# worldbench/lidarcrafter

Measured on AMD Instinct MI355X. Metric: denoising-steps/sec, nuScenes 32×1024 range image, 1/2/4/8 GPU, higher is better.
Workload: dtype f16x2-split MFMA, fp32 accumulate (fp32-class accuracy)

## Files before the change

### include/lidarcrafter_hip.h

```cpp
#ifndef LIDARCRAFTER_HIP_H
#define LIDARCRAFTER_HIP_H

#include <stdint.h>

#ifdef __cplusplus
extern "C" {
#endif

#define LC_OK 0
#define LC_EINVAL (-1)
#define LC_EUNSUP (-2)

typedef void* lc_stream_t;

int lc_abi_version(void);
int lc_device_arch(char* buf, int buflen);
int lc_load_code_objects(void);

int64_t lc_packed_conv_weight_elems(int Co, int Ci, int ks);
int lc_pack_conv_weight(const float* w_oihw, float* wp, int Co, int Ci, int ks, lc_stream_t s);
int lc_conv2d_ring_fwd(const float* x, int64_t x_bs, const float* wp, const float* bias,
                       const float* res, int64_t res_bs, float* y, int64_t y_bs,
                       int B, int Ci, int Co, int H, int W, int ks, float out_scale,
                       int tile_cfg , lc_stream_t s);
// ... 142 lines not shown
int lc_hdit_rmsnorm_fwd(const float* x, int64_t x_bs, int64_t x_cs, const float* f, int64_t f_bs, int mode, float* y,
                        int64_t y_bs, int64_t y_cs, int B, int C, int L, float eps, lc_stream_t s);
int lc_hdit_geglu_fwd(const float* x, int64_t x_bs, float* y, int64_t y_bs, int B, int mid, int L, lc_stream_t s);
int lc_hdit_qk_prep_fwd(float* q, int64_t q_bs, int64_t q_cs, float* k, int64_t k_bs, int64_t k_cs, const float* scale,
                        const float* cos_t, const float* sin_t, int B, int heads, int d, int L, lc_stream_t s);
int lc_hdit_na_fwd(const lc_cm_operand* q, const lc_cm_operand* k, const lc_cm_operand* v, float* o, int64_t o_bs,
                   int64_t o_hs, int64_t o_cs, int B, int heads, int d, int h, int w, int kh, int kw, float scale,
                   lc_stream_t s);
int lc_hdit_space_to_depth_fwd(const float* in, int64_t in_bs, float* out, int64_t out_bs, int B, int C, int H, int W,
                               int P1, int P2, lc_stream_t s);
int lc_hdit_depth_to_space_fwd(const float* in, int64_t in_bs, float* out, int64_t out_bs, const float* skip,
                               int64_t skip_bs, const float* alpha, int B, int C, int h, int w, int P1, int P2,
                               lc_stream_t s);
int lc_hdit_tokenize_fwd(const float* x, int64_t x_bs, const float* wt, const float* pe, float* y, int64_t y_bs, int B,
                         int Cin, int C, int H, int W, int P, lc_stream_t s);
int lc_hdit_fourier_fwd(const float* t, const float* freqs, float* y, int M, int half, lc_stream_t s);
int lc_hdit_na_train_fwd(const lc_cm_operand* q, const lc_cm_operand* k, const lc_cm_operand* v, float* o,
                         int64_t o_bs, int64_t o_hs, int64_t o_cs, float* lse, int B, int heads, int d, int h, int w,
                         int kh, int kw, float scale, lc_stream_t s);
int lc_hdit_rmsnorm_bwd(const float* x, int64_t x_bs, int64_t x_cs, const float* f, int64_t f_bs, int mode,
                        const float* dy, int64_t dy_bs, int64_t dy_cs, float* dx, int64_t dx_bs, int64_t dx_cs,
                        float* rs, float* df, int64_t df_bs, int B, int C, int L, float eps, lc_stream_t s);
int lc_hdit_geglu_bwd(const float* x, int64_t x_bs, const float* dy, int64_t dy_bs, float* dx, int64_t dx_bs, int B,
                      int mid, int L, lc_stream_t s);
int lc_hdit_qk_prep_bwd(const float* q, int64_t q_bs, int64_t q_cs, const float* k, int64_t k_bs, int64_t k_cs,
                        const float* gq, int64_t gq_bs, int64_t gq_cs, const float* gk, int64_t gk_bs, int64_t gk_cs,
                        float* dq, int64_t dq_bs, int64_t dq_cs, float* dk, int64_t dk_bs, int64_t dk_cs,
                        const float* scale, const float* cos_t, const float* sin_t, double* part, float* dscale, int B,
                        int heads, int d, int L, lc_stream_t s);
int lc_hdit_na_bwd(const lc_cm_operand* q, const lc_cm_operand* k, const lc_cm_operand* v, const lc_cm_operand* o,
                   const lc_cm_operand* dout, const float* lse, float* dsum, float* dq, float* dk, float* dv, int B,
                   int heads, int d, int h, int w, int kh, int kw, float scale, lc_stream_t s);
int lc_hdit_lerp_bwd(const float* dout, int64_t dout_bs, const float* y, int64_t y_bs, const float* skip,
                     int64_t skip_bs, const float* alpha, float* dskip, int64_t dskip_bs, float* dy, int64_t dy_bs,
                     float* dalpha, int B, int C, int h, int w, int P1, int P2, lc_stream_t s);
int64_t lc_groupnorm_jvp_partials_elems(int B, int C, int H, int W, int G);
int lc_groupnorm_jvp_stats(const float* x, int64_t x_bs, const float* dx, int64_t dx_bs, double* partials, int B, int C,
                           int H, int W, int G, lc_stream_t s);
int lc_groupnorm_jvp_apply_train(const float* x, int64_t x_bs, const float* dx, int64_t dx_bs, const double* partials,
                                 const float* gamma, const float* beta, const float* scale, const float* shift,
                                 const float* dscale, const float* dshift, int64_t ss_bs, float* y, int64_t y_bs,
                                 float* dy, int64_t dy_bs, int B, int C, int H, int W, int G, float eps, int act_silu,
                                 float* mean_rstd_out, float* amax_out, float* damax_out, lc_stream_t s);
int lc_qk_norm_cm_jvp(const float* x, int64_t x_bs, int64_t x_cs, const float* dx, int64_t dx_bs, int64_t dx_cs,
                      const float* g, float* y, int64_t y_bs, int64_t y_cs, float* dy, int64_t dy_bs, int64_t dy_cs,
                      int B, int heads, int d, int L, lc_stream_t s);
int64_t lc_qk_norm_cm_bwd_partials(int B, int heads, int L);
int lc_qk_norm_cm_bwd(const float* x, int64_t x_bs, int64_t x_cs, const float* gy, int64_t gy_bs, int64_t gy_cs,
                      const float* g, float* gx, int64_t gx_bs, int64_t gx_cs, double* dg_partials, float* dg, int B,
                      int heads, int d, int L, lc_stream_t s);
int lc_attention_jvp_fwd(const float* q, const float* k, const float* v, const float* dq, const float* dk,
                         const float* dv, float* o, float* lse, float* dout, int BH, int Lq, int Lk, int dqk, int dv_ch,
                         float scale, lc_stream_t s);
int lc_conv1x1_f16x2_ps_qkv_fwd(const void* x_split, const void* wp_hi, const void* wp_lo, const float* bias, float* q,
                                int64_t q_bs, void* kv, int B, int Ci, int C, int H, int W, int Lk1, const float* wmeta,
                                lc_conv_range* range, lc_stream_t s);
int64_t lc_attention_units_elems(int B, int heads, int Lk0, int Lk1);
int lc_attention_pack_units(const lc_cm_operand* src, void* kv, int B, int heads, int L, int Lk0, int Lk1, int d,
                            int cb0, int key0, int which, lc_stream_t s);
int lc_attention_units_fwd(const lc_cm_operand* q, const lc_cm_operand* q_pos, const void* kv, float* o,
                           int64_t o_bs, int64_t o_hs, int64_t o_cs, int B, int heads, int Lq, int Lk0, int Lk1,
                           int dqk, int dpos, int dv, float scale, lc_stream_t s);
int lc_attention_train_fwd(const float* q, const float* k, const float* v, float* o, float* lse, int BH, int Lq,
                           int Lk, int dqk, int dv, float scale, int f16x2, float* qkv_amax, lc_stream_t s);
int lc_attention_bwd(const float* q, const float* k, const float* v, const float* o, const float* dout,
                     const float* lse, float* dsum_scratch, float* dq, float* dk, float* dv, int BH, int Lq, int Lk,
                     int dqk, int dv_ch, float scale, lc_stream_t s);
int lc_attention_bwd_f16x2(const float* q, const float* k, const float* v, const float* o, const float* dout,
                           const float* lse, float* dsum_scratch, float* dq, float* dk, float* dv, int BH, int Lq,
                           int Lk, int dqk, int dv_ch, float scale, const float* qkv_amax, lc_stream_t s);

int lc_pstep_fwd(const float* x_t, int64_t xt_bs, const float* pred, int64_t pred_bs,
                 const float* noise, int64_t noise_bs, const float* coef, float* x_s,
                 int64_t xs_bs, int B, int64_t n, int objective, int mode, lc_stream_t s);

int lc_gate_bias_act(const float* x, int64_t x_bs, const float* gate_logit, const float* bias,
                     int64_t gb_bs, const float* res, int64_t res_bs, float* y, int64_t y_bs,
                     int B, int C, int N, int act, lc_stream_t s);

int64_t lc_fir_down2_split_units(int B, int C, int H, int W);
int lc_fir_down2_prefilter_split(const float* x, int64_t x_bs, void* y_split, int B, int C, int H, int W,
                                 lc_conv_range* range, lc_stream_t s);
int64_t lc_conv2d_ring_s2_stats_slots(int Ho, int Wo);
int lc_conv2d_ring_s2_f16x2_ps_fwd(const void* x_split, const void* wp_hi, const void* wp_lo, const float* bias, float* y,
                                   int64_t y_bs, int B, int Ci, int Co, int Ho, int Wo, float out_scale,
                                   float* gn_ostats_out, int gn_ostats_unit, const float* wmeta, lc_conv_range* range,
                                   lc_stream_t s);

int64_t lc_calibrate_mfma_f16(const void* operands, int blocks, int iters, float* sink, lc_stream_t s);
int lc_calibrate_stream_copy(const float* src, float* dst, int64_t n, lc_stream_t s);

int lc_copy_strided(const float* x, int64_t x_bs, float* y, int64_t y_bs, int B, int64_t n,
                    lc_stream_t s);
int lc_add_scale(const float* a, int64_t a_bs, const float* b, int64_t b_bs, float* y,
                 int64_t y_bs, int B, int64_t n, float scale, lc_stream_t s);

int64_t lc_conv2d_ring_wgrad_scratch_elems(int B, int Ci, int Co, int H, int W, int ks);
int lc_conv2d_ring_wgrad(const float* x, int64_t x_bs, const float* dy, int64_t dy_bs, float* scratch,
                         float* dw , float* dbias , int B, int Ci,
                         int Co, int H, int W, int ks, int accumulate, lc_stream_t s);
int lc_conv2d_ring_wgrad_f16x2(const float* x, int64_t x_bs, const float* dy, int64_t dy_bs,
                               const lc_conv_range* x_range, const lc_conv_range* dy_range,
                               float* scratch, float* dw, float* dbias, int B, int Ci, int Co, int H,
                               int W, int ks, int accumulate, lc_stream_t s);
int lc_groupnorm_meanrstd(const float* x, int64_t x_bs, const double* partials, float* mean_rstd,
                          int B, int C, int H, int W, int G, float eps, lc_stream_t s);
int lc_groupnorm_bwd(const float* x, int64_t x_bs, const float* dy, int64_t dy_bs,
                     const float* mean_rstd, const float* gamma, const float* beta, const float* scale,
                     const float* shift, int64_t ss_bs, double* rows, float* dx, int64_t dx_bs, int B,
                     int C, int H, int W, int G, int act_silu, lc_stream_t s);
int lc_groupnorm_bwd_train(const float* x, int64_t x_bs, const float* dy, int64_t dy_bs,
                           const float* mean_rstd, const float* gamma, const float* beta, const float* scale,
                           const float* shift, int64_t ss_bs, double* rows, float* dx, int64_t dx_bs,
                           float* dgamma, float* dbeta, float* dscale, float* dshift, int B, int C, int H, int W,
                           int G, int act_silu, float* amax_out, lc_stream_t s);

int lc_bev_occupancy_accumulate(const float* pts, int pt_stride, int N, float x0, float x1, float y0,
                                float y1, float voxel, int min_bound_x, int min_bound_y, int nx,
                                int ny, int stamp, int32_t* stamps, float* grid, lc_stream_t s);
int64_t lc_sparse_quantize_scratch_bytes(int N, int D);
int lc_sparse_quantize(const float* coords, int N, int D, float vx, float vy, float vz, void* scratch,
                       int32_t* out_coords, int64_t* out_index, int64_t* out_inverse,
                       uint64_t* out_count, lc_stream_t s);

int lc_project_points(const float* points, int N, int H, int W, double fov_up_deg,
                      double fov_down_deg, float min_depth, float max_depth, uint64_t* zbuf,
                      float* image, int32_t* winner, int32_t* cells, int elev_f64, lc_stream_t s);
int lc_project_workspace_init(uint64_t* zbuf, int n_cells, lc_stream_t s);
int lc_project_points_ws(const float* points, int N, int H, int W, double fov_up_deg,
                         double fov_down_deg, float min_depth, float max_depth, uint64_t* zbuf,
                         float* image, int32_t* winner, int32_t* cells, int elev_f64, lc_stream_t s);
int lc_project_points_f64(const double* points, int N, int H, int W, double fov_up_deg,
                          double fov_down_deg, double min_depth, double max_depth, uint64_t* zbuf,
                          int32_t* winner, float* image, lc_stream_t s);

int lc_points_in_boxes_mask(const float* boxes, int n_boxes, const float* pts, int n_pts,
                            float margin, int32_t* out_mask, lc_stream_t s);
int lc_points_in_boxes_index(const float* boxes, const float* pts, int B, int n_boxes, int n_pts,
                             float margin, int32_t* out_idx, lc_stream_t s);

int lc_range_postprocess(const float* sample, int64_t sample_bs, const float* ray_angles,
                         float* out, int B, int H, int W, int depth_format, float min_depth,
                         float max_depth, lc_stream_t s);
int lc_condition_preprocess(const float* condition_mask, int64_t cm_bs, float* out, int64_t out_bs,
                            int B, int H, int W, int num_classes, int depth_format,
                            float min_depth, float max_depth, lc_stream_t s);

int64_t lc_layout_scratch_bytes(int B, int T);
int lc_layout_condition(const void* boxes, int boxes_f64, int box_stride, const int32_t* n_valid,
                        int B, int T, int H, int W, double fov_up_deg, double fov_down_deg,
                        void* scratch, float* corners_2d, float* condition_mask,
                        float* loss_weight_map, lc_stream_t s);

int lc_roiaware_pool3d_fwd(const float* rois, const float* pts, const float* pts_feature,
                           int n_boxes, int n_pts, int channels, int out_x, int out_y, int out_z,
                           int max_pts_each_voxel, int pool_method, int32_t* pts_mask_scratch,
                           int32_t* pts_idx_of_voxels, int32_t* argmax, float* pooled,
                           lc_stream_t s);
int lc_roiaware_pool3d_bwd(const int32_t* pts_idx_of_voxels, const int32_t* argmax,
                           const float* grad_out, float* grad_in, int n_boxes, int channels,
                           int out_x, int out_y, int out_z, int max_pts_each_voxel,
                           int pool_method, lc_stream_t s);

int lc_transform_points(const float* pts, int N, const double* T16_host, float* out, lc_stream_t s);
int lc_transform_points_f64(const float* pts, int N, const double* T16_host, int rot_f32,
                            double* out, lc_stream_t s);
// ... 79 lines not shown
```

### lidarcrafter_amd/_lib.py

```python
from __future__ import annotations

import ctypes as C
import os

from .build import LIB

i32, i64, f32, f64, vp = C.c_int, C.c_int64, C.c_float, C.c_double, C.c_void_p


class CmOperand(C.Structure):
    _fields_ = [("p", vp), ("bs", i64), ("hs", i64), ("cs", i64)]


_op = C.POINTER(CmOperand)


class OctStats(C.Structure):
    _fields_ = [("p", vp), ("channels", i32), ("slots", i32), ("unit", i32)]


_os = C.POINTER(OctStats)


class GnStatsInput(C.Structure):
# ... 35 lines not shown
    "lc_groupnorm_apply_split": (i32, [vp, i64, vp, vp, vp, vp, vp, i64, vp, i32, i32, i32, i32, i32,
                                       f32, i32, vp, vp]),
    "lc_groupnorm_apply_os_split": (i32, [vp, i64, _os, _os, vp, vp, vp, vp, i64, vp, i32, i32, i32,
                                          i32, i32, f32, i32, vp, vp]),
    "lc_conv1x1_f16x2_ps_fwd": (i32, [vp, vp, vp, vp, vp, i64, vp, i64, i32, i32, i32, i32, i32, f32, vp, vp, vp]),
    "lc_conv2d_ring_f16x2_ps_fwd": (i32, [vp, vp, vp, vp, vp, i64, vp, i64, i32, i32, i32, i32, i32,
                                          f32, i32, vp, i32, vp, i32, vp, vp, vp]),
    "lc_range_from_tensor": (i32, [vp, i64, i32, i64, vp, vp]),
    "lc_splitk_stats_slots": (i64, [i32, i32]),
    "lc_splitk_reduce": (i32, [vp, i32, vp, vp, i64, vp, i64, i32, i32, i32, i32, f32, vp, vp]),
    "lc_conv2d_ring_f16x2_stats_slots": (i64, [i32, i32, i32, i32, i32, i32, i32]),
    "lc_groupnorm_coeffs": (i32, [vp, i64, vp, vp, vp, vp, vp, i64, vp, i32, i32, i32, i32, i32,
                                  i32, f32, vp]),
    "lc_groupnorm_partials_elems": (i64, [i32, i32, i32, i32, i32]),
    "lc_groupnorm_stats": (i32, [vp, i64, vp, i32, i32, i32, i32, i32, vp]),
    "lc_groupnorm_apply": (i32, [vp, i64, vp, vp, vp, vp, vp, i64, vp, i64, i32, i32, i32, i32,
                                 i32, f32, i32, vp]),
    "lc_groupnorm_apply_train": (i32, [vp, i64, vp, vp, vp, vp, vp, i64, vp, i64, i32, i32, i32, i32,
                                       i32, f32, i32, vp, vp, vp]),
    "lc_groupnorm_apply_os": (i32, [vp, i64, _os, _os, vp, vp, vp, vp, i64, vp, i64, i32, i32, i32,
                                    i32, i32, f32, i32, vp]),
    "lc_conv2d_ring_wgrad_scratch_elems": (i64, [i32, i32, i32, i32, i32, i32]),
    "lc_conv2d_ring_wgrad": (i32, [vp, i64, vp, i64, vp, vp, vp, i32, i32, i32, i32, i32, i32, i32, vp]),
    "lc_conv2d_ring_wgrad_f16x2": (i32, [vp, i64, vp, i64, vp, vp, vp, vp, vp, i32, i32, i32, i32, i32,
                                         i32, i32, vp]),
    "lc_groupnorm_meanrstd": (i32, [vp, i64, vp, vp, i32, i32, i32, i32, i32, f32, vp]),
    "lc_groupnorm_bwd": (i32, [vp, i64, vp, i64, vp, vp, vp, vp, vp, i64, vp, vp, i64, i32, i32, i32,
                               i32, i32, i32, vp]),
    "lc_groupnorm_bwd_train": (i32, [vp, i64, vp, i64, vp, vp, vp, vp, vp, i64, vp, vp, i64, vp, vp, vp, vp,
                                     i32, i32, i32, i32, i32, i32, vp, vp]),
    "lc_resample2x_fwd": (i32, [vp, i64, vp, i64, i32, i32, i32, i32, i32, vp]),
    "lc_resample2x_stats_slots": (i64, [i32, i32, i32]),
    "lc_resample2x_stats_fwd": (i32, [vp, i64, vp, i64, i32, i32, i32, i32, i32, vp, vp]),
    "lc_linear_fwd": (i32, [vp, vp, vp, vp, i32, i32, i32, i32, i32, vp]),
    "lc_sinusoid_fwd": (i32, [vp, vp, i32, i32, f32, vp]),
    "lc_attention_fwd": (i32, [_op, _op, _op, _op, _op, _op, _op, _op, vp, i64, i64, i64,
                               i32, i32, i32, i32, i32, i32, i32, i32, f32, vp]),
    "lc_attention_f16x2_fwd": (i32, [_op, _op, _op, _op, _op, _op, _op, _op, vp, i64, i64, i64,
                                     i32, i32, i32, i32, i32, i32, i32, i32, f32, vp]),
    "lc_conv1x1_f16x2_ps_qkv_fwd": (i32, [vp, vp, vp, vp, vp, i64, vp, i32, i32, i32, i32, i32, i32, vp, vp, vp]),
    "lc_groupnorm_coeffs_os": (i32, [_os, _os, vp, vp, vp, vp, i64, vp, i32, i32, i32, i32, f32, vp]),
    "lc_resample2x_pair_fwd": (i32, [vp, i64, vp, i32, vp, i64, vp, i64, i32, i32, i32, i32, i32, vp]),
    "lc_split_act_fwd": (i32, [vp, i64, vp, i32, i32, i32, i32, vp, vp]),
    "lc_up2_combine9_stats_slots": (i64, [i32, i32]),
    "lc_up2_combine9_fwd": (i32, [vp, i64, vp, vp, i64, i32, i32, i32, i32, vp, vp]),
    "lc_up2_combine9_xup_fwd": (i32, [vp, i64, vp, vp, i64, vp, i64, vp, i64, i32, i32, i32, i32, vp, vp]),
    "lc_attention_units_elems": (i64, [i32, i32, i32, i32]),
    "lc_attention_pack_units": (i32, [_op, vp, i32, i32, i32, i32, i32, i32, i32, i32, i32, vp]),
    "lc_attention_units_fwd": (i32, [_op, _op, vp, vp, i64, i64, i64, i32, i32, i32, i32, i32, i32, i32, i32, f32, vp]),
    "lc_qk_norm_cm_fwd": (i32, [vp, i64, i64, vp, i64, i64, vp, vp, i32, i32, i32, i32, vp]),
    "lc_flow_step_fwd": (i32, [vp, i64, vp, i64, vp, vp, i64, i32, i64, vp]),
    "lc_hdit_rmsnorm_fwd": (i32, [vp, i64, i64, vp, i64, i32, vp, i64, i64, i32, i32, i32, f32, vp]),
    "lc_hdit_geglu_fwd": (i32, [vp, i64, vp, i64, i32, i32, i32, vp]),
    "lc_hdit_qk_prep_fwd": (i32, [vp, i64, i64, vp, i64, i64, vp, vp, vp, i32, i32, i32, i32, vp]),
    "lc_hdit_na_fwd": (i32, [_op, _op, _op, vp, i64, i64, i64, i32, i32, i32, i32, i32, i32, i32, f32, vp]),
    "lc_hdit_space_to_depth_fwd": (i32, [vp, i64, vp, i64, i32, i32, i32, i32, i32, i32, vp]),
    "lc_hdit_depth_to_space_fwd": (i32, [vp, i64, vp, i64, vp, i64, vp, i32, i32, i32, i32, i32, i32, vp]),
    "lc_hdit_tokenize_fwd": (i32, [vp, i64, vp, vp, vp, i64, i32, i32, i32, i32, i32, i32, vp]),
    "lc_hdit_fourier_fwd": (i32, [vp, vp, vp, i32, i32, vp]),
    "lc_hdit_na_train_fwd": (i32, [_op, _op, _op, vp, i64, i64, i64, vp, i32, i32, i32, i32, i32, i32, i32, f32, vp]),
    "lc_hdit_rmsnorm_bwd": (i32, [vp, i64, i64, vp, i64, i32, vp, i64, i64, vp, i64, i64, vp, vp, i64, i32, i32, i32,
                                  f32, vp]),
    "lc_hdit_geglu_bwd": (i32, [vp, i64, vp, i64, vp, i64, i32, i32, i32, vp]),
    "lc_hdit_qk_prep_bwd": (i32, [vp, i64, i64, vp, i64, i64, vp, i64, i64, vp, i64, i64, vp, i64, i64, vp, i64, i64,
                                  vp, vp, vp, vp, vp, i32, i32, i32, i32, vp]),
    "lc_hdit_na_bwd": (i32, [_op, _op, _op, _op, _op, vp, vp, vp, vp, vp, i32, i32, i32, i32, i32, i32, i32, f32, vp]),
    "lc_hdit_lerp_bwd": (i32, [vp, i64, vp, i64, vp, i64, vp, vp, i64, vp, i64, vp, i32, i32, i32, i32, i32, i32, vp]),
    "lc_groupnorm_jvp_partials_elems": (i64, [i32, i32, i32, i32, i32]),
    "lc_groupnorm_jvp_stats": (i32, [vp, i64, vp, i64, vp, i32, i32, i32, i32, i32, vp]),
    "lc_groupnorm_jvp_apply_train": (i32, [vp, i64, vp, i64, vp, vp, vp, vp, vp, vp, vp, i64, vp, i64, vp, i64,
                                           i32, i32, i32, i32, i32, f32, i32, vp, vp, vp, vp]),
    "lc_qk_norm_cm_jvp": (i32, [vp, i64, i64, vp, i64, i64, vp, vp, i64, i64, vp, i64, i64, i32, i32, i32, i32, vp]),
    "lc_qk_norm_cm_bwd_partials": (i64, [i32, i32, i32]),
    "lc_qk_norm_cm_bwd": (i32, [vp, i64, i64, vp, i64, i64, vp, vp, i64, i64, vp, vp, i32, i32, i32, i32, vp]),
    "lc_attention_jvp_fwd": (i32, [vp, vp, vp, vp, vp, vp, vp, vp, vp, i32, i32, i32, i32, i32, f32, vp]),
    "lc_attention_train_fwd": (i32, [vp, vp, vp, vp, vp, i32, i32, i32, i32, i32, f32, i32, vp, vp]),
    "lc_attention_bwd": (i32, [vp, vp, vp, vp, vp, vp, vp, vp, vp, vp, i32, i32, i32, i32, i32, f32, vp]),
    "lc_attention_bwd_f16x2": (i32, [vp, vp, vp, vp, vp, vp, vp, vp, vp, vp, i32, i32, i32, i32, i32, f32, vp, vp]),
    "lc_pstep_fwd": (i32, [vp, i64, vp, i64, vp, i64, vp, vp, i64, i32, i64, i32, i32, vp]),
    "lc_gate_bias_act": (i32, [vp, i64, vp, vp, i64, vp, i64, vp, i64, i32, i32, i32, i32, vp]),
    "lc_fir_down2_split_units": (i64, [i32, i32, i32, i32]),
    "lc_fir_down2_prefilter_split": (i32, [vp, i64, vp, i32, i32, i32, i32, vp, vp]),
    "lc_conv2d_ring_s2_stats_slots": (i64, [i32, i32]),
    "lc_conv2d_ring_s2_f16x2_ps_fwd": (i32, [vp, vp, vp, vp, vp, i64, i32, i32, i32, i32, i32, f32, vp, i32, vp, vp, vp]),
    "lc_calibrate_mfma_f16": (i64, [vp, i32, i32, vp, vp]),
    "lc_calibrate_stream_copy": (i32, [vp, vp, i64, vp]),
    "lc_copy_strided": (i32, [vp, i64, vp, i64, i32, i64, vp]),
    "lc_add_scale": (i32, [vp, i64, vp, i64, vp, i64, i32, i64, f32, vp]),
    "lc_project_points": (i32, [vp, i32, i32, i32, f64, f64, f32, f32, vp, vp, vp, vp, i32, vp]),
    "lc_project_workspace_init": (i32, [vp, i32, vp]),
    "lc_project_points_ws": (i32, [vp, i32, i32, i32, f64, f64, f32, f32, vp, vp, vp, vp, i32, vp]),
    "lc_project_points_f64": (i32, [vp, i32, i32, i32, f64, f64, f64, f64, vp, vp, vp, vp]),
    "lc_range_postprocess": (i32, [vp, i64, vp, vp, i32, i32, i32, i32, f32, f32, vp]),
    "lc_condition_preprocess": (i32, [vp, i64, vp, i64, i32, i32, i32, i32, i32, f32, f32, vp]),
    "lc_layout_scratch_bytes": (i64, [i32, i32]),
    "lc_layout_condition": (i32, [vp, i32, i32, vp, i32, i32, i32, i32, f64, f64, vp, vp, vp, vp, vp]),
    "lc_roiaware_pool3d_fwd": (i32, [vp, vp, vp, i32, i32, i32, i32, i32, i32, i32, i32, vp, vp, vp,
                                     vp, vp]),
    "lc_roiaware_pool3d_bwd": (i32, [vp, vp, vp, vp, i32, i32, i32, i32, i32, i32, i32, vp]),
    "lc_points_in_boxes_mask": (i32, [vp, i32, vp, i32, f32, vp, vp]),
    "lc_points_in_boxes_mask4": (i32, [vp, i32, vp, i32, f32, vp, vp, vp]),
    "lc_transform_points": (i32, [vp, i32, C.POINTER(C.c_double), vp, vp]),
    "lc_transform_points_f64": (i32, [vp, i32, C.POINTER(C.c_double), i32, vp, vp]),
    "lc_image_to_points": (i32, [vp, i64, vp, vp, i32, i32, f32, f32, f32, vp, vp, vp]),
    "lc_bev_occupancy_accumulate": (i32, [vp, i32, i32, f32, f32, f32, f32, f32, i32, i32, i32, i32,
                                          i32, vp, vp, vp]),
    "lc_sparse_quantize_scratch_bytes": (i64, [i32, i32]),
    "lc_sparse_quantize": (i32, [vp, i32, i32, f32, f32, f32, vp, vp, vp, vp, vp, vp]),
    "lc_bev_histogram": (i32, [vp, i32, i32, vp, i32, f32, f32, vp, vp, vp]),
    "lc_rbf_partials_elems": (i64, [i32, i32]),
    "lc_rbf_kernel_sum": (i32, [vp, vp, i32, i32, i32, f32, vp, vp]),
    "lc_chamfer3d_fwd": (i32, [vp, vp, i32, i32, i32, vp, vp, vp, vp, vp]),
    "lc_chamfer2d_fwd": (i32, [vp, vp, i32, i32, i32, vp, vp, vp, vp, vp]),
    "lc_bev_grid_supported": (i32, [i32, i32]),
    "lc_bev_occupancy_bits": (i32, [vp, i32, vp, i32, i64, f32, f32, f32, f32, f32, i32, i32, i32, i32, vp, vp, vp]),
    "lc_bev_cell_lists": (i32, [vp, i32, i32, i32, vp, vp, vp]),
    "lc_bev_distance_transform": (i32, [vp, i32, i32, i32, vp, vp, i32, vp]),
    "lc_bev_pair_sums": (i32, [vp, vp, i32, vp, i32, i32, vp, vp]),
    "lc_bev_chamfer_combine": (i32, [vp, vp, vp, vp, i32, i32, i64, i32, i32, i32, vp, vp, vp, i64, vp]),
    "lc_emd_scratch_bytes": (i64, [i32, i32]),
    "lc_emd_fwd": (i32, [vp, vp, i32, i32, f32, i32, i32, vp, vp, vp, vp]),
    "lc_compact_scratch_elems": (i64, [i32]),
    "lc_compact_points": (i32, [vp, vp, i32, i32, vp, vp, vp, vp, vp]),
    "lc_points_in_boxes_index": (i32, [vp, vp, i32, i32, i32, f32, vp, vp]),
    "lc_skinny_parts": (i64, [i32, i32, i32]),
    "lc_skinny_gemm_fwd": (i32, [_rs, i32, vp, vp, i32, i32, i32, i32, vp]),
    "lc_skinny_combine_fwd": (i32, [vp, i32, vp, i32, vp, i64, vp, vp, i64, vp, i64, i32, i32, vp]),
    "lc_rowprep_fwd": (i32, [_rs, i32, vp, i64, i32, i32, i32, f32, vp, vp, i32, vp]),
    "lc_graph_pool_fwd": (i32, [vp, i64, i32, i32, vp, vp, vp, i64, i32, i32, vp]),
    "lc_time_embed_fwd": (i32, [vp, vp, vp, i32, i32, vp]),
    "lc_pointnet_trunk_scratch_elems": (i64, [i32, i32]),
    "lc_pointnet_trunk_fwd": (i32, [vp, i64, vp, vp, vp, vp, vp, vp, vp, i32, vp, i64, i32, i32, vp, vp]),
    "lc_spconv_hash_bytes": (i64, [i32]),
    "lc_spconv_hash_build": (i32, [vp, i32, i32, i32, vp, i64, vp]),
    "lc_spconv_map": (i32, [vp, i32, i32, i32, vp, i32, vp, vp]),
    "lc_spconv_fwd": (i32, [vp, i64, vp, i32, vp, vp, vp, i64, vp, i64, i32, i32, i32, i32, i32, i32, vp]),
    "lc_spconv_sector_means": (i32, [vp, i64, vp, vp, i32, i32, vp, f32, vp, vp]),
}

_lib = None
ABI_VERSION = 5


class HipLibraryMissing(RuntimeError):
    pass


def lib() -> C.CDLL:
    global _lib
    if _lib is None:
        path = os.environ.get("LC_HIP_LIB", LIB)
        if not os.path.exists(path):
            raise HipLibraryMissing(
                f"{path} not found: run `python -m lidarcrafter_amd.build` "
                "(or __graft_entry__.build()). There is no CPU fallback for the hot path.")
        handle = C.CDLL(path)
        for name, (res, args) in SIGNATURES.items():
            fn = getattr(handle, name)
            fn.restype, fn.argtypes = res, args
        if handle.lc_abi_version() != ABI_VERSION:
            raise HipLibraryMissing("ABI version mismatch, rebuild the library")
        _lib = handle
    return _lib


_lib_p1 = None
# ... 26 lines not shown
```

### lidarcrafter_amd/csrc/conv_f16x2_s2.hip

```cpp
#include "conv_f16x2_common.h"

using namespace lcconv;

namespace {

#include "conv_f16x2_ps.h"

typedef _Float16 half8_s2 __attribute__((ext_vector_type(8)));

__global__ __launch_bounds__(256) void fir_down2_prefilter_split_kernel(
    const float* __restrict__ x, long long x_bs, half8_s2* __restrict__ ysp, int C8, int H, int W, int nstrip, int strip_len,
    lc_conv_range* range) {
    const int Wh = W >> 1;
    const int i = blockIdx.x * 256 + threadIdx.x;
    const int c8 = blockIdx.y;
    const int b = blockIdx.z / nstrip, strip = blockIdx.z - b * nstrip;
    const float xs = range->x_scale, seen = range->amax_scaled;
    float am = 0.f;
    if (i < Wh) {
        const long long HW = (long long)H * W;
        const float* xb = x + b * x_bs + (long long)c8 * 8 * HW;
        const int R = H + 3;
        half8_s2* yh = ysp + ((long long)b * 2 * C8 + c8) * R * W;
        half8_s2* yl = yh + (long long)C8 * R * W;
// ... 212 lines not shown
    const int co_wave = co0 + wco * 32 + 4 * kh;
    float bias_r[16];
#pragma unroll
    for (int r = 0; r < 16; ++r) {
        const int co = co_wave + (r & 3) + 8 * (r >> 2);
        bias_r[r] = (a.bias && co < a.Co) ? a.bias[co] : 0.0f;
    }
    asm volatile("s_waitcnt vmcnt(0)" ::: "memory");
    __syncthreads();

    const int nchunk = a.Cib / CB;
    int xb = 0;
    for (int ch = 0; ch < nchunk; ++ch) {
        const int wb = ch & 1;
        const bool more = ch + 1 < nchunk;
        using I0 = std::integral_constant<int, 0>;
        using I1 = std::integral_constant<int, 1>;
        using I2 = std::integral_constant<int, 2>;
        using I3 = std::integral_constant<int, 3>;
        using NO = std::false_type;
        using YES = std::true_type;
        if constexpr (TPB == 1) {
            iteration(I0{}, I0{}, YES{}, xb, wb, ch + 1, more); xb ^= 1;
        } else if constexpr (TPB == 2) {
            iteration(I0{}, I1{}, NO{}, xb, wb, ch, true); xb ^= 1;
            iteration(I1{}, I0{}, YES{}, xb, wb, ch + 1, more); xb ^= 1;
        } else {
            iteration(I0{}, I1{}, NO{}, xb, wb, ch, true); xb ^= 1;
            iteration(I1{}, I2{}, NO{}, xb, wb, ch, true); xb ^= 1;
            iteration(I2{}, I3{}, NO{}, xb, wb, ch, true); xb ^= 1;
            iteration(I3{}, I0{}, YES{}, xb, wb, ch + 1, more); xb ^= 1;
        }
    }

    const unsigned HW4 = (unsigned)HW * 4u;
    const __amdgpu_buffer_rsrc_t rs_yb = __builtin_amdgcn_make_buffer_rsrc((void*)(a.y + (long long)b * a.y_bs), 0, (unsigned)a.Co * HW4, 0x00020000);
    const bool quads = a.ounit == 4;
    const int ush = quads ? 2 : 3;
    __amdgpu_buffer_rsrc_t rs_o = rs_yb;
    if constexpr (EMIT_STATS)
        rs_o = __builtin_amdgcn_make_buffer_rsrc((void*)(a.ostats + (long long)b * (a.Co >> ush) * a.oslots), 0,
                                                 (unsigned)(a.Co >> ush) * (unsigned)a.oslots * 16u, 0x00020000);
#pragma unroll
    for (int t = 0; t < TPB; ++t) {
        const int gh = h0 + t, gw = w0 + wpx * 32 + l31;
        const bool pok = gh < H && gw < W;
        const unsigned vo = pok ? (unsigned)(co_wave * HW + gh * W + gw) * 4u : OOB;
        const float brow = (gh == 0 ? 0.875f : 1.0f) + (gh == H - 1 ? 0.875f : 1.0f) - 1.0f;
        float st_p[4], st_s[4], st_q[4];
#pragma unroll
        for (int r = 0; r < 16; ++r) {
            const int cor = (r & 3) + 8 * (r >> 2);
            const float v = (acc[t][r] * out_unscale + bias_r[r] * brow) * a.out_scale;
            __builtin_amdgcn_raw_buffer_store_b32(__builtin_bit_cast(unsigned, v), rs_yb, co_wave + cor < a.Co ? vo : OOB,
                                                  (unsigned)cor * HW4, LC_DEF_AUX);
            if constexpr (EMIT_STATS) {
                const int m = r >> 2;
                if ((r & 3) == 0) { st_p[m] = __builtin_amdgcn_readlane(pok ? v : 0.0f, 0); st_s[m] = 0.f; st_q[m] = 0.f; }
                const float d = pok ? v - st_p[m] : 0.0f;
                st_s[m] += d;
                st_q[m] = fmaf(d, d, st_q[m]);
            }
        }
        if constexpr (EMIT_STATS) {
            const int nvalid = __popcll(__ballot(pok) & 0xFFFFFFFFull);
            const int slot = (gh * a.tiles_w + tw_i) * 2 + wpx;
            const bool mine = quads ? (lane & 31) >= 28 : lane >= 60;
            const float nv = (float)((quads ? 4 : 8) * nvalid);
#pragma unroll
            for (int m = 0; m < 4; ++m) {
                const int co_oct = co0 + wco * 32 + 8 * m;
                const float sh = half_sum_to_lane31_63(st_s[m]), qh = half_sum_to_lane31_63(st_q[m]);
                const float sf = dpp_add<0x143, 0xC>(sh), qf = dpp_add<0x143, 0xC>(qh);
                const int ent = quads ? (co_oct >> 2) + (lane >> 5) : (co_oct >> 3);
                const unsigned eo = (mine && co_oct < a.Co && gh < H)
                                        ? ((unsigned)ent * (unsigned)a.oslots + (unsigned)slot) * 16u + 4u * (lane & 3)
                                        : OOB;
                store_entry_4lanes(rs_o, st_p[m], nv, quads ? sh : sf, quads ? qh : qf, eo);
            }
        }
    }
}

using S2Cfg = HCfg<2, 2, 1, 1, 1, 64, 3>;

}

extern "C" int64_t lc_conv2d_ring_s2_stats_slots(int Ho, int Wo) {
    if (Ho <= 0 || Wo <= 0 || Wo % S2Cfg::TW_) return 0;
    return (int64_t)Ho * (Wo / S2Cfg::TW_) * S2Cfg::WPX_;
}

extern "C" int64_t lc_fir_down2_split_units(int B, int C, int H, int W) {
    if (B <= 0 || C <= 0 || C % 8 || H <= 0 || W <= 0) return 0;
    return (int64_t)B * 2 * (C / 8) * (H + 3) * W;
}

extern "C" int lc_fir_down2_prefilter_split(const float* x, int64_t x_bs, void* y_split, int B, int C, int H, int W,
                                            lc_conv_range* range, lc_stream_t s) {
    if (!x || !y_split || !range || B <= 0 || C <= 0 || H <= 0 || W <= 0) return LC_EINVAL;
    if (C % 16 || H % 2 || H < 4 || W % 128) return LC_EUNSUP;
    if ((reinterpret_cast<uintptr_t>(x) & 7) || (x_bs & 1)) return LC_EUNSUP;
    int strip_len = 8;
    static const int strip_env = [] { const char* e = getenv("LC_PF_STRIP"); return e ? atoi(e) : 0; }();
    if (strip_env > 0) strip_len = strip_env;
    const int nstrip = (H + 1 + strip_len - 1) / strip_len;
    if ((long long)B * nstrip > 65535) return LC_EUNSUP;
    dim3 grid((W / 2 + 255) / 256, C / 8, B * nstrip);
    hipLaunchKernelGGL(fir_down2_prefilter_split_kernel, grid, dim3(256), 0, lc_s(s), x, (long long)x_bs,
                       reinterpret_cast<half8_s2*>(y_split), C / 8, H, W, nstrip, strip_len, range);
    return lc_launch_status();
}

extern "C" int lc_conv2d_ring_s2_f16x2_ps_fwd(const void* x_split, const void* wp_hi, const void* wp_lo, const float* bias,
                                              float* y, int64_t y_bs, int B, int Ci, int Co, int Ho, int Wo, float out_scale,
                                              float* gn_ostats_out, int gn_ostats_unit, const float* wmeta,
                                              lc_conv_range* range, lc_stream_t s) {
    using C = S2Cfg;
    if (!x_split || !wp_hi || !wp_lo || !y || !wmeta || !range || B <= 0 || Ci <= 0 || Co <= 0 || Ho <= 0 || Wo <= 0)
        return LC_EINVAL;
    if (Ci % 16 || Ho < 2 || Wo % C::TW_) return LC_EUNSUP;
    const long long plane_units = (long long)(Ci / 8) * (2 * Ho + 3) * (2 * Wo);
    if (2 * plane_units * 16 >= (1ll << 31) || (long long)Co * Ho * Wo * 4 >= (1ll << 31)) return LC_EUNSUP;
    ConvArgsH a;
    a.x = nullptr; a.wh = (const half8*)wp_hi; a.wl = (const half8*)wp_lo; a.bias = bias; a.res = nullptr;
    a.y = y; a.x_bs = 0; a.res_bs = 0; a.y_bs = y_bs;
    a.range = range; a.wmeta = wmeta;
    a.B = B; a.Ci = Ci; a.Co = Co; a.H = Ho; a.W = Wo;
    a.Cib = Ci / 8; a.Cop = (Co + 63) / 64 * 64;
    if (a.wl != a.wh + (long long)9 * a.Cib * a.Cop) return LC_EINVAL;
    a.xsp = (const half8*)x_split; a.xsp_c8 = Ci / 8; a.xsp_bs = 2 * plane_units;
    a.part = nullptr; a.ksplit = 0;
    a.out_scale = out_scale;
    a.gn = nullptr; a.Cgn = 0; a.gn_silu = 0;
    a.gs = lc_gn_stats_input{nullptr, 0, 0, 0.f, nullptr, nullptr, nullptr, nullptr, 0, nullptr, nullptr};
    a.seg[0] = a.seg[1] = ConvArgsH::OctSeg{nullptr, 0, 0, 3};
    a.ostats = nullptr; a.oslots = 0; a.ounit = 8;
    if (gn_ostats_out) {
        if (Co % 8 || (gn_ostats_unit != 8 && gn_ostats_unit != 4)) return LC_EUNSUP;
        a.oslots = (int)lc_conv2d_ring_s2_stats_slots(Ho, Wo);
        a.ostats = reinterpret_cast<f32x4*>(gn_ostats_out);
        a.ounit = gn_ostats_unit;
    }
    a.tiles_h = Ho; a.tiles_w = Wo / C::TW_;
    const int ncot = (Co + C::BN - 1) / C::BN;
    const long long n_tiles = (long long)B * a.tiles_h * a.tiles_w * ncot;
    int tpb = 1;
    while (tpb < 4 && a.tiles_h % (tpb * 2) == 0 && n_tiles / (tpb * 2) >= 256) tpb *= 2;
    a.tpb = tpb; a.vert = 1;
    dim3 grid(B * a.tiles_h * a.tiles_w / tpb, ncot);
    a.xcd = (grid.x % 8 == 0 && grid.x >= 16) ? 1 : 0;
    static const int form_env = [] { const char* e = getenv("LC_S2_FORM"); return e ? atoi(e) : 2; }();
    if (form_env == 1) {
        if (a.ostats) hipLaunchKernelGGL((conv_f16x2_ps_kernel<C, true, true>), grid, dim3(C::NT), 0, lc_s(s), a);
        else hipLaunchKernelGGL((conv_f16x2_ps_kernel<C, false, true>), grid, dim3(C::NT), 0, lc_s(s), a);
        return lc_launch_status();
    }
#define LC_S2_LAUNCH(T)                                                                                          \
    do {                                                                                                         \
        if (a.ostats) hipLaunchKernelGGL((conv_s2_shared_w_kernel<T, true>), grid, dim3(256), 0, lc_s(s), a);    \
        else hipLaunchKernelGGL((conv_s2_shared_w_kernel<T, false>), grid, dim3(256), 0, lc_s(s), a);            \
    } while (0)
    if (tpb == 4) LC_S2_LAUNCH(4);
    else if (tpb == 2) LC_S2_LAUNCH(2);
    else LC_S2_LAUNCH(1);
#undef LC_S2_LAUNCH
    return lc_launch_status();
}

LC_TOUCH_TU(conv_f16x2_s2, fir_down2_prefilter_split_kernel)
```

Measured before the change: 286.0.

## Add row-group stride-2 conv kernel sharing input rows across four output rows

Adds a new stride-2 ring conv kernel in which each block computes four output rows (one per wave). It stages the shared 2*RG+3 input rows and all nine weight taps in LDS per channel chunk, double-buffered with LDS DMA, and packs two taps per 32x32x16 MFMA step. The aim is to cut redundant input and weight loads compared with the per-row shared-weight kernel. The new form becomes the default whenever the planner picks four tiles per block, and a runtime form switch plus a query API are exported. A devtools report script for comparing traces is also added. The cost is a large LDS footprint per block and one block per CU occupancy.

```diff
diff --git a/devtools/s2_tile_report.py b/devtools/s2_tile_report.py
--- /dev/null
+++ b/devtools/s2_tile_report.py
@@ -0,0 +1,39 @@
+import csv, glob, json, os, sys
+from collections import defaultdict
+O = sys.argv[1]
+print("headline (ms_per_step, median of 10 sweeps of 20 steps):")
+for who in ("parent", "new"):
+    vals = []
+    for i in (1, 2, 3):
+        try:
+            d = json.load(open(f"{O}/head_{who}_{i}.json"))
+            vals.append((d.get("ms_per_step"), d.get("value")))
+        except Exception as e:
+            vals.append(("ERR", str(e)[:60]))
+    print(" ", who, vals)
+for who in ("parent", "new"):
+    fs = glob.glob(f"{O}/trace_{who}/**/*kernel_trace.csv", recursive=True)
+    if not fs:
+        print("no trace for", who); continue
+    rows = [r for r in csv.DictReader(open(fs[0])) if "conv_s2_" in r["Kernel_Name"]]
+    rows.sort(key=lambda r: int(r["Start_Timestamp"]))
+    rows = rows[-60:]
+    pos = defaultdict(list)
+    for i, r in enumerate(rows):
+        pos[i % 3].append((int(r["End_Timestamp"]) - int(r["Start_Timestamp"])) / 1e3)
+    names = [rows[i]["Kernel_Name"][:70] for i in range(min(3, len(rows)))]
+    print("trace", who, "launches", len(rows), {k: round(sum(v) / len(v), 2) for k, v in pos.items()},
+          "min", {k: round(min(v), 2) for k, v in pos.items()}, names)
+for who in ("parent", "new"):
+    fs = glob.glob(f"{O}/pmc_{who}/**/*counter_collection.csv", recursive=True)
+    if not fs:
+        print("no pmc for", who); continue
+    acc = defaultdict(lambda: defaultdict(list))
+    order = []
+    for r in csv.DictReader(open(fs[0])):
+        if "conv_s2_" not in r["Kernel_Name"]:
+            continue
+        key = (r["Kernel_Name"][:60], r.get("Grid_Size", ""))
+        acc[key][r["Counter_Name"]].append(float(r["Counter_Value"]))
+    for key, d in acc.items():
+        print("pmc", who, key, {c: round(sum(v) / len(v), 1) for c, v in d.items()}, "n", {c: len(v) for c, v in d.items()})
diff --git a/include/lidarcrafter_hip.h b/include/lidarcrafter_hip.h
--- a/include/lidarcrafter_hip.h
+++ b/include/lidarcrafter_hip.h
@@ -248,6 +248,8 @@
 int lc_fir_down2_prefilter_split(const float* x, int64_t x_bs, void* y_split, int B, int C, int H, int W,
                                  lc_conv_range* range, lc_stream_t s);
 int64_t lc_conv2d_ring_s2_stats_slots(int Ho, int Wo);
+int lc_conv2d_ring_s2_form(int form);
+int lc_conv2d_ring_s2_form_of(int B, int Co, int Ho, int Wo);
 int lc_conv2d_ring_s2_f16x2_ps_fwd(const void* x_split, const void* wp_hi, const void* wp_lo, const float* bias, float* y,
                                    int64_t y_bs, int B, int Ci, int Co, int Ho, int Wo, float out_scale,
                                    float* gn_ostats_out, int gn_ostats_unit, const float* wmeta, lc_conv_range* range,
diff --git a/lidarcrafter_amd/_lib.py b/lidarcrafter_amd/_lib.py
--- a/lidarcrafter_amd/_lib.py
+++ b/lidarcrafter_amd/_lib.py
@@ -141,6 +141,8 @@
     "lc_fir_down2_split_units": (i64, [i32, i32, i32, i32]),
     "lc_fir_down2_prefilter_split": (i32, [vp, i64, vp, i32, i32, i32, i32, vp, vp]),
     "lc_conv2d_ring_s2_stats_slots": (i64, [i32, i32]),
+    "lc_conv2d_ring_s2_form": (i32, [i32]),
+    "lc_conv2d_ring_s2_form_of": (i32, [i32, i32, i32, i32]),
     "lc_conv2d_ring_s2_f16x2_ps_fwd": (i32, [vp, vp, vp, vp, vp, i64, i32, i32, i32, i32, i32, f32, vp, i32, vp, vp, vp]),
     "lc_calibrate_mfma_f16": (i64, [vp, i32, i32, vp, vp]),
     "lc_calibrate_stream_copy": (i32, [vp, vp, i64, vp]),
diff --git a/lidarcrafter_amd/csrc/conv_f16x2_s2.hip b/lidarcrafter_amd/csrc/conv_f16x2_s2.hip
--- a/lidarcrafter_amd/csrc/conv_f16x2_s2.hip
+++ b/lidarcrafter_amd/csrc/conv_f16x2_s2.hip
@@ -318,8 +318,268 @@
     }
 }
 
+struct S2RowGroup {
+    static constexpr int RG = 4;
+    static constexpr int NTAP = 9, NSTEP = 5;
+    static constexpr int BN = 64, TW = 64;
+    static constexpr int XW = 2 * TW + 1;
+    static constexpr int XR = 2 * RG + 3;
+    static constexpr int SLOT_TOP = 2 * RG + 1, SLOT_BOT = 2 * RG + 2;
+    __host__ __device__ static constexpr int slot_of(int h0, int t, int ky, int Ho) {
+        return (h0 + t == 0 && ky == 2) ? SLOT_TOP : ((h0 + t == Ho - 1 && ky == 0) ? SLOT_BOT : 2 * t + ky);
+    }
+    __host__ __device__ static constexpr int row_of_slot(int h0, int slot, int Ho) {
+        if (slot < SLOT_TOP) return 2 * h0 + slot <= 2 * Ho ? 2 * h0 + slot : -1;
+        if (slot == SLOT_TOP) return h0 == 0 ? 2 * Ho + 1 : -1;
+        return (h0 <= Ho - 1 && Ho - 1 < h0 + RG) ? 2 * Ho + 2 : -1;
+    }
+};
+
+template <bool EMIT_STATS>
+__global__ __launch_bounds__(256, 1) void conv_s2_rowgroup_kernel(ConvArgsH a) {
+    using G = S2RowGroup;
+    constexpr int RG = G::RG, NTAP = G::NTAP, NSTEP = G::NSTEP, BN = G::BN, TW = G::TW, XW = G::XW, XR = G::XR;
+    constexpr int XU = XR * XW, WU = NTAP * BN;
+    constexpr int NWV = 4;
+    constexpr int NXI = (XU + 63) / 64, NWI = (WU + 63) / 64;
+    constexpr int XS = NXI * 64, WS = NWI * 64;
+    constexpr int KX = (2 * NXI + NWV - 1) / NWV, KW = (2 * NWI + NWV - 1) / NWV;
+    constexpr int NSLOT = KX + KW, SPT = (NSLOT + NSTEP - 1) / NSTEP;
+    constexpr unsigned OOB = 0x80000000u;
+    __shared__ half8 xlds[2][2 * XS];
+    __shared__ half8 wlds[2][2 * WS];
+    __shared__ half8 dummy[64];
+    const int tid = threadIdx.x, lane = tid & 63;
+    const int wave = __builtin_amdgcn_readfirstlane(tid >> 6);
+    const int kh = lane >> 5, l31 = lane & 31;
+
+    int bx = blockIdx.x;
+    if (a.xcd) bx = (bx & 7) * (gridDim.x >> 3) + (bx >> 3);
+    const int gh_ = (a.tiles_h + RG - 1) / RG;
+    const int tw_i = bx % a.tiles_w; bx /= a.tiles_w;
+    const int h0 = (bx % gh_) * RG; bx /= gh_;
+    const int b = bx;
+    const int w0 = tw_i * TW;
+    const int co0 = blockIdx.y * BN;
+    const int H = a.H, W = a.W, HW = H * W;
+    const int C8 = a.xsp_c8;
+    const int XROWS = 2 * H + 3, XCOLS = 2 * W;
+    const float out_unscale = a.range->x_unscale * a.wmeta[1];
+
+    const unsigned xbytes = 2u * (unsigned)C8 * (unsigned)(XROWS * XCOLS) * 16u;
+    const __amdgpu_buffer_rsrc_t rs_x = __builtin_amdgcn_make_buffer_rsrc((void*)(a.xsp + (long long)b * a.xsp_bs), 0, xbytes, 0x00020000);
+    const unsigned wplane = (unsigned)(NTAP * a.Cib) * (unsigned)a.Cop;
+    const __amdgpu_buffer_rsrc_t rs_w = __builtin_amdgcn_make_buffer_rsrc((void*)a.wh, 0, 2u * wplane * 16u, 0x00020000);
+
+    unsigned vx[KX];
+    int lx[KX];
+#pragma unroll
+    for (int k = 0; k < KX; ++k) {
+        const int j = wave + k * NWV;
+        const int plane = j / NXI, e = (j - plane * NXI) * 64 + lane;
+        const int slot = e / XW, c = e - slot * XW;
+        int col;
+        if (c <= TW) { col = w0 + c; col = col >= W ? col - W : col; }
+        else col = W + w0 + (c - TW - 1);
+        const int row = G::row_of_slot(h0, slot, H);
+        const bool ok = j < 2 * NXI && e < XU && row >= 0;
+        lx[k] = j < 2 * NXI ? plane * XS + (j - plane * NXI) * 64 : -1;
+        vx[k] = ok ? (unsigned)((plane * C8 * XROWS + row) * XCOLS + col) * 16u : OOB;
+    }
+    unsigned vw[KW];
+    int lw[KW];
+#pragma unroll
+    for (int k = 0; k < KW; ++k) {
+        const int j = wave + k * NWV;
+        const int plane = j / NWI, e = (j - plane * NWI) * 64 + lane;
+        const int tap = e / BN, cu = e - tap * BN;
+        lw[k] = j < 2 * NWI ? plane * WS + (j - plane * NWI) * 64 : -1;
+        vw[k] = (j < 2 * NWI && e < WU) ? ((unsigned)(tap * a.Cib * a.Cop + co0 + cu) + plane * wplane) * 16u : OOB;
+    }
+    const unsigned x_chunk = (unsigned)(XROWS * XCOLS) * 16u;
+    const unsigned w_chunk = (unsigned)a.Cop * 16u;
+    auto dma_slot = [&](int buf, int k, int ch) {
+        if (k < KX) {
+            half8* dst = lx[k] >= 0 ? &xlds[buf][lx[k]] : dummy;
+            lds_dma16(rs_x, (lds_vptr)dst, vx[k], (unsigned)ch * x_chunk);
+        } else {
+            half8* dst = lw[k - KX] >= 0 ? &wlds[buf][lw[k - KX]] : dummy;
+            lds_dma16(rs_w, (lds_vptr)dst, vw[k - KX], (unsigned)ch * w_chunk);
+        }
+    };
+
+    f32x16 acc[2][2];
+#pragma unroll
+    for (int g = 0; g < 2; ++g)
+#pragma unroll
+        for (int f = 0; f < 2; ++f)
+#pragma unroll
+            for (int r = 0; r < 16; ++r) acc[g][f][r] = 0.0f;
+    int xo[NSTEP], wo[NSTEP];
+#pragma unroll
+    for (int p = 0; p < NSTEP; ++p) {
+        const int tap = 2 * p + kh < NTAP ? 2 * p + kh : NTAP - 1;
+        const int dy = tap / 3, dx = tap - dy * 3;
+        xo[p] = G::slot_of(h0, wave, dy, H) * XW + (dx == 1 ? TW + 1 : (dx == 2 ? 1 : 0)) + l31;
+        wo[p] = tap * BN + l31;
+    }
+    const bool pad_lane = kh != 0;
+
+    auto chunk = [&](int cur, int nch, bool issue_next) {
+        const half8* cxh = &xlds[cur][0];
+        const half8* cxl = cxh + XS;
+        const half8* cwh = &wlds[cur][0];
+        const half8* cwl = cwh + WS;
+        half8 ah[2][2], al[2][2], bh[2][2], bl[2][2];
+        auto fetch = [&](int p, int s) {
+#pragma unroll
+            for (int g = 0; g < 2; ++g) {
+                ah[s][g] = cwh[wo[p] + g * 32];
+                al[s][g] = cwl[wo[p] + g * 32];
+                bh[s][g] = cxh[xo[p] + g * 32];
+                bl[s][g] = cxl[xo[p] + g * 32];
+            }
+            if (p == NSTEP - 1) {
+                const half8 z = {0, 0, 0, 0, 0, 0, 0, 0};
+#pragma unroll
+                for (int g = 0; g < 2; ++g) {
+                    ah[s][g] = pad_lane ? z : ah[s][g];
+                    al[s][g] = pad_lane ? z : al[s][g];
+                }
+            }
+        };
+        fetch(0, 0);
+#pragma unroll
+        for (int p = 0; p < NSTEP; ++p) {
+            const int s = p & 1;
+            __builtin_amdgcn_sched_barrier(0);
+            if (p + 1 < NSTEP) fetch(p + 1, s ^ 1);
+            if (issue_next) {
+#pragma unroll
+                for (int q = 0; q < SPT; ++q)
+                    if (p * SPT + q < NSLOT) dma_slot(cur ^ 1, p * SPT + q, nch);
+            }
+            __builtin_amdgcn_sched_barrier(0);
+            if (LC_F16X2_TERMS & 2) {
+#pragma unroll
+                for (int g = 0; g < 2; ++g)
+#pragma unroll
+                    for (int f = 0; f < 2; ++f) acc[g][f] = __builtin_amdgcn_mfma_f32_32x32x16_f16(al[s][g], bh[s][f], acc[g][f], 0, 0, 0);
+            }
+            if (LC_F16X2_TERMS & 4) {
+#pragma unroll
+                for (int g = 0; g < 2; ++g)
+#pragma unroll
+                    for (int f = 0; f < 2; ++f) acc[g][f] = __builtin_amdgcn_mfma_f32_32x32x16_f16(ah[s][g], bl[s][f], acc[g][f], 0, 0, 0);
+            }
+#pragma unroll
+            for (int g = 0; g < 2; ++g)
+#pragma unroll
+                for (int f = 0; f < 2; ++f) acc[g][f] = __builtin_amdgcn_mfma_f32_32x32x16_f16(ah[s][g], bh[s][f], acc[g][f], 0, 0, 0);
+        }
+        __builtin_amdgcn_sched_barrier(0);
+        asm volatile("s_waitcnt vmcnt(0)" ::: "memory");
+        __syncthreads();
+    };
+
+#pragma unroll
+    for (int k = 0; k < NSLOT; ++k) dma_slot(0, k, 0);
+    asm volatile("s_waitcnt vmcnt(0)" ::: "memory");
+    __syncthreads();
+
+    const int nchunk = a.Cib;
+    for (int ch = 0; ch < nchunk; ++ch) chunk(ch & 1, ch + 1, ch + 1 < nchunk);
+
+    const unsigned HW4 = (unsigned)HW * 4u;
+    const __amdgpu_buffer_rsrc_t rs_yb = __builtin_amdgcn_make_buffer_rsrc((void*)(a.y + (long long)b * a.y_bs), 0, (unsigned)a.Co * HW4, 0x00020000);
+    const bool quads = a.ounit == 4;
+    const int ush = quads ? 2 : 3;
+    __amdgpu_buffer_rsrc_t rs_o = rs_yb;
+    if constexpr (EMIT_STATS)
+        rs_o = __builtin_amdgcn_make_buffer_rsrc((void*)(a.ostats + (long long)b * (a.Co >> ush) * a.oslots), 0,
+                                                 (unsigned)(a.Co >> ush) * (unsigned)a.oslots * 16u, 0x00020000);
+    const int gh = h0 + wave;
+    const float brow = (gh == 0 ? 0.875f : 1.0f) + (gh == H - 1 ? 0.875f : 1.0f) - 1.0f;
+#pragma unroll
+    for (int g = 0; g < 2; ++g) {
+        const int co_wave = co0 + g * 32 + 4 * kh;
+        float bias_r[16];
+#pragma unroll
+        for (int r = 0; r < 16; ++r) {
+            const int co = co_wave + (r & 3) + 8 * (r >> 2);
+            bias_r[r] = (a.bias && co < a.Co) ? a.bias[co] : 0.0f;
+        }
+#pragma unroll
+        for (int f = 0; f < 2; ++f) {
+            const int gw = w0 + f * 32 + l31;
+            const bool pok = gh < H && gw < W;
+            const unsigned vo = pok ? (unsigned)(co_wave * HW + gh * W + gw) * 4u : OOB;
+            float st_p[4], st_s[4], st_q[4];
+#pragma unroll
+            for (int r = 0; r < 16; ++r) {
+                const int cor = (r & 3) + 8 * (r >> 2);
+                const float v = (acc[g][f][r] * out_unscale + bias_r[r] * brow) * a.out_scale;
+                __builtin_amdgcn_raw_buffer_store_b32(__builtin_bit_cast(unsigned, v), rs_yb, co_wave + cor < a.Co ? vo : OOB,
+                                                      (unsigned)cor * HW4, LC_DEF_AUX);
+                if constexpr (EMIT_STATS) {
+                    const int m = r >> 2;
+                    if ((r & 3) == 0) { st_p[m] = __builtin_amdgcn_readlane(pok ? v : 0.0f, 0); st_s[m] = 0.f; st_q[m] = 0.f; }
+                    const float d = pok ? v - st_p[m] : 0.0f;
+                    st_s[m] += d;
+                    st_q[m] = fmaf(d, d, st_q[m]);
+                }
+            }
+            if constexpr (EMIT_STATS) {
+                const int nvalid = __popcll(__ballot(pok) & 0xFFFFFFFFull);
+                const int slot = (gh * a.tiles_w + tw_i) * 2 + f;
+                const bool mine = quads ? (lane & 31) >= 28 : lane >= 60;
+                const float nv = (float)((quads ? 4 : 8) * nvalid);
+#pragma unroll
+                for (int m = 0; m < 4; ++m) {
+                    const int co_oct = co0 + g * 32 + 8 * m;
+                    const float sh = half_sum_to_lane31_63(st_s[m]), qh = half_sum_to_lane31_63(st_q[m]);
+                    const float sf = dpp_add<0x143, 0xC>(sh), qf = dpp_add<0x143, 0xC>(qh);
+                    const int ent = quads ? (co_oct >> 2) + (lane >> 5) : (co_oct >> 3);
+                    const unsigned eo = (mine && co_oct < a.Co && gh < H)
+                                            ? ((unsigned)ent * (unsigned)a.oslots + (unsigned)slot) * 16u + 4u * (lane & 3)
+                                            : OOB;
+                    store_entry_4lanes(rs_o, st_p[m], nv, quads ? sh : sf, quads ? qh : qf, eo);
+                }
+            }
+        }
+    }
+}
+
 using S2Cfg = HCfg<2, 2, 1, 1, 1, 64, 3>;
 
+}
+
+static int& s2_form_switch() {
+    static int form = [] { const char* e = getenv("LC_S2_FORM"); const int f = e ? atoi(e) : 3; return f >= 1 && f <= 4 ? f : 3; }();
+    return form;
+}
+
+static int s2_plan(int B, int Co, int Ho, int Wo, int* tpb_out) {
+    const int ncot = (Co + S2Cfg::BN - 1) / S2Cfg::BN;
+    const long long n_tiles = (long long)B * Ho * (Wo / S2Cfg::TW_) * ncot;
+    int tpb = 1;
+    while (tpb < 4 && Ho % (tpb * 2) == 0 && n_tiles / (tpb * 2) >= 256) tpb *= 2;
+    *tpb_out = tpb;
+    const int sw = s2_form_switch();
+    if (sw <= 2) return sw;
+    return (sw == 4 || tpb == S2RowGroup::RG) ? 3 : 2;
+}
+
+extern "C" int lc_conv2d_ring_s2_form(int form) {
+    const int prev = s2_form_switch();
+    if (form >= 1 && form <= 4) s2_form_switch() = form;
+    return prev;
+}
+
+extern "C" int lc_conv2d_ring_s2_form_of(int B, int Co, int Ho, int Wo) {
+    if (B <= 0 || Co <= 0 || Ho < 2 || Wo <= 0 || Wo % S2Cfg::TW_) return 0;
+    int tpb;
+    return s2_plan(B, Co, Ho, Wo, &tpb);
 }
 
 extern "C" int64_t lc_conv2d_ring_s2_stats_slots(int Ho, int Wo) {
@@ -380,14 +640,20 @@
     }
     a.tiles_h = Ho; a.tiles_w = Wo / C::TW_;
     const int ncot = (Co + C::BN - 1) / C::BN;
-    const long long n_tiles = (long long)B * a.tiles_h * a.tiles_w * ncot;
     int tpb = 1;
-    while (tpb < 4 && a.tiles_h % (tpb * 2) == 0 && n_tiles / (tpb * 2) >= 256) tpb *= 2;
+    const int form = s2_plan(B, Co, Ho, Wo, &tpb);
+    if (form == 3) {
+        a.tpb = S2RowGroup::RG; a.vert = 1;
+        dim3 grid(B * ((Ho + S2RowGroup::RG - 1) / S2RowGroup::RG) * a.tiles_w, ncot);
+        a.xcd = (grid.x % 8 == 0 && grid.x >= 16) ? 1 : 0;
+        if (a.ostats) hipLaunchKernelGGL((conv_s2_rowgroup_kernel<true>), grid, dim3(256), 0, lc_s(s), a);
+        else hipLaunchKernelGGL((conv_s2_rowgroup_kernel<false>), grid, dim3(256), 0, lc_s(s), a);
+        return lc_launch_status();
+    }
     a.tpb = tpb; a.vert = 1;
     dim3 grid(B * a.tiles_h * a.tiles_w / tpb, ncot);
     a.xcd = (grid.x % 8 == 0 && grid.x >= 16) ? 1 : 0;
-    static const int form_env = [] { const char* e = getenv("LC_S2_FORM"); return e ? atoi(e) : 2; }();
-    if (form_env == 1) {
+    if (form == 1) {
         if (a.ostats) hipLaunchKernelGGL((conv_f16x2_ps_kernel<C, true, true>), grid, dim3(C::NT), 0, lc_s(s), a);
         else hipLaunchKernelGGL((conv_f16x2_ps_kernel<C, false, true>), grid, dim3(C::NT), 0, lc_s(s), a);
         return lc_launch_status();
```

New measurement: 285.9 (median of 3 runs). No clear change (-0.0%).
